# devarshpatel1506/Real-Time-Student-Attendance-System

Hardware: AMD Instinct MI355X
Metric: swipes/sec (fused BF.EXISTS+PFADD) at 1/2/4/8 GPUs; % of HBM peak (higher is better)
Workload: dtype u64; 1 GPU; c3-1B-10M-100kkeys; students=10000000, hll_keys_total=100000, hll_keys_this_gpu=100000, key_ownership=MurmurHash64A(key name, 0) mod world (distributed.KeyMap), id_bytes=8, parallelism=dp1 (key-sharded, Bloom replicated), k1_variant=partitioned, layout=offsets, streams=1, input=routed to the key owners at ingest, launch=host, answers=written (1 B per swipe)

## Files before the change

include/sketch.h:

```cpp
#ifndef SKETCH_H
#define SKETCH_H

#include <stddef.h>
#include <stdint.h>

#ifdef __cplusplus
extern "C" {
#endif

#define SKE_OK 0
#define SKE_EINVAL -1
#define SKE_ENOMEM -2
#define SKE_EHIP -3
#define SKE_ENOFILTER -4
#define SKE_EEXISTS -5
#define SKE_EFULL -6
#define SKE_ERANGE -7
#define SKE_EBADRATE -8
#define SKE_EBADCAP -9
#define SKE_EBADEXP -10
#define SKE_EBADHLL -11
#define SKE_ETOOLONG -12
#define SKE_EBUSY -13
#define SKE_ECMSNOKEY -14
// ... 261 lines not shown
    const uint32_t *slot;
    const uint8_t *bytes;
    const uint32_t *offs;
    uint32_t width;
    uint64_t n;
    uint8_t *out_valid;
} ske_swipe_batch;
int ske_swipes_many_async(ske_ctx *ctx, uint32_t fid, const ske_swipe_batch *batches,
                          uint32_t nbatch, uint32_t branches);
int ske_swipes_stats(ske_ctx *ctx, uint32_t fid, const uint8_t *bytes, const uint32_t *offs,
                     uint64_t n, uint64_t *probes, uint64_t *nvalid);
int ske_swipes_variant(ske_ctx *ctx, uint32_t fid);
int ske_set_option(ske_ctx *ctx, const char *name, int64_t value);
#define SKE_PASS_KINDS 9
int ske_pass_times(ske_ctx *ctx, double *ms_out, uint64_t *count_out, int reset);

typedef struct {
    uint8_t *status;
    uint32_t *id_start, *id_len, *lec_start, *lec_len, *ts_start, *ts_len;
    int32_t *day;
    uint64_t *kh;
} ske_ingest_cols_t;
int ske_ingest_parse(ske_ctx *ctx, const uint8_t *msgs, const uint32_t *moffs, uint64_t n,
                     int day_form, const ske_ingest_cols_t *cols);
int ske_keytab_lookup(ske_ctx *ctx, const ske_ingest_cols_t *cols, uint64_t n, uint32_t *slot_dev,
                      uint64_t *nmiss);
int ske_keytab_insert(ske_ctx *ctx, const uint64_t *kh_host, const uint32_t *slots_host, uint64_t n);
int ske_keytab_clear(ske_ctx *ctx);
int ske_ingest_swipes(ske_ctx *ctx, uint32_t fid, const uint8_t *msgs,
                      const ske_ingest_cols_t *cols, uint64_t n, uint8_t *valid_dev,
// ... 31 lines not shown
```

real-time-student-attendance-system_amd/_lib.py:

```python
from __future__ import annotations

import ctypes as C
import os

_HERE = os.path.dirname(os.path.abspath(__file__))
LIB_PATH = os.environ.get("SKE_LIB") or os.path.join(_HERE, "csrc", "libsketch.so")
HEADER_PATH = os.path.join(os.path.dirname(_HERE), "include", "sketch.h")

SKE_OK = 0
SKE_EINVAL = -1
SKE_ENOMEM = -2
SKE_EHIP = -3
SKE_ENOFILTER = -4
SKE_EEXISTS = -5
SKE_EFULL = -6
SKE_ERANGE = -7
SKE_EBADRATE = -8
SKE_EBADCAP = -9
SKE_EBADEXP = -10
SKE_EBADHLL = -11
SKE_ETOOLONG = -12
SKE_EBUSY = -13
SKE_ECMSNOKEY = -14
SKE_ECMSEXISTS = -15
# ... 199 lines not shown
    "ske_swipes_fixed_async": (C.c_int, [_CTX, C.c_uint32, _u32p, _u8p, C.c_uint32, C.c_uint64,
                                         _u8p]),
    "ske_swipes_many_async": (C.c_int, [_CTX, C.c_uint32, _vp, C.c_uint32, C.c_uint32]),
    "ske_swipes_fixed_bits": (C.c_int, [_CTX, C.c_uint32, _u32p, _u8p, C.c_uint32, C.c_uint64, _u8p, C.c_int]),
    "ske_route_swipes": (C.c_int, [_CTX, _u8p, C.c_uint32, _u32p, C.c_uint64, C.c_uint32, _u32p, _u32p,
                                   C.c_uint32, _u8p, _u32p, _u32p, _u64p]),
    "ske_route_swipes_cap_async": (C.c_int, [_CTX, _u8p, C.c_uint32, _u32p, C.c_uint64, C.c_uint32, _u32p,
                                             C.c_uint32, C.c_uint32, _u32p, _u8p, _u32p, _u32p, _u32p]),
    "ske_route_return_async": (C.c_int, [_CTX, _u8p, _u32p, C.c_uint64, _u8p]),
    "ske_route_slots_async": (C.c_int, [_CTX, _u32p, C.c_uint64, _u32p, C.c_uint32, C.c_uint32, _u32p]),
    "ske_swipes_stats": (C.c_int, [_CTX, C.c_uint32, _u8p, _u32p, C.c_uint64,
                                   C.POINTER(C.c_uint64), C.POINTER(C.c_uint64)]),
    "ske_swipes_variant": (C.c_int, [_CTX, C.c_uint32]),
    "ske_set_option": (C.c_int, [_CTX, C.c_char_p, C.c_int64]),
    "ske_pass_times": (C.c_int, [_CTX, C.POINTER(C.c_double), C.POINTER(C.c_uint64), C.c_int]),
    "ske_ingest_parse": (C.c_int, [_CTX, _u8p, _u32p, C.c_uint64, C.c_int, C.POINTER(IngestCols)]),
    "ske_keytab_lookup": (C.c_int, [_CTX, C.POINTER(IngestCols), C.c_uint64, _u32p,
                                    C.POINTER(C.c_uint64)]),
    "ske_keytab_insert": (C.c_int, [_CTX, _u64p, _u32p, C.c_uint64]),
    "ske_keytab_clear": (C.c_int, [_CTX]),
    "ske_ingest_swipes": (C.c_int, [_CTX, C.c_uint32, _u8p, C.POINTER(IngestCols), C.c_uint64, _u8p,
                                    C.POINTER(C.c_uint64)]),
    "ske_ingest_times": (C.c_int, [_CTX, _u8p, C.POINTER(IngestCols), C.c_uint64, _vp]),
    "ske_ingest_dense": (C.c_int, [_CTX, _u8p, C.POINTER(IngestCols), C.c_uint64, _u8p, _vp,
                                   C.POINTER(IngestDense), C.c_uint64, C.POINTER(C.c_uint64),
                                   C.POINTER(C.c_uint64)]),
    "ske_capture_begin": (C.c_int, [_CTX]),
    "ske_capture_end": (C.c_int, [_CTX, C.POINTER(C.c_void_p)]),
    "ske_graph_launch": (C.c_int, [_CTX, _vp]),
    "ske_graph_free": (C.c_int, [_CTX, _vp]),
# ... 75 lines not shown
```

real-time-student-attendance-system_amd/csrc/sketch_api_ctx.cpp:

```cpp
#include <stdlib.h>
#include <string.h>

#include "sketch_ctx.h"

using namespace ske;

namespace ske {

void *stage_buf(ske_ctx *c, StageSlot slot, size_t bytes, int *rc) {
    if (bytes < 64) bytes = 64;
    if (c->stg_cap[slot] < bytes) {
        if (c->stg[slot]) (void)hipFree(c->stg[slot]);
        c->stg[slot] = nullptr;
        c->stg_cap[slot] = 0;
        size_t want = bytes + bytes / 4 + 256;
        hipError_t e = hipMalloc(&c->stg[slot], want);
        if (e != hipSuccess) {
            c->last_hip = std::string("hipMalloc(staging): ") + hipGetErrorString(e);
            *rc = SKE_ENOMEM;
            return nullptr;
        }
        c->stg_cap[slot] = want;
    }
    return c->stg[slot];
// ... 388 lines not shown
        }
        mark_recycle(c, m);
    }
    c->marks.clear();
    for (int i = 0; i < kPassKinds; i++) {
        ms[i] = c->pass_ms[i];
        count[i] = c->pass_n[i];
        if (reset) {
            c->pass_ms[i] = 0;
            c->pass_n[i] = 0;
        }
    }
    return SKE_OK;
}

int ske_device_alloc(ske_ctx *c, uint64_t bytes, void **out) {
    if (!c || !out) return SKE_EINVAL;
    hipError_t e = hipMalloc(out, bytes ? bytes : 16);
    if (e != hipSuccess) {
        c->last_hip = std::string("hipMalloc: ") + hipGetErrorString(e);
        return SKE_ENOMEM;
    }
    return SKE_OK;
}

int ske_device_free(ske_ctx *c, void *p) {
    if (!c) return SKE_EINVAL;
    HIPCHK(c, hipFree(p));
    return SKE_OK;
}
// ... 12 lines not shown
int ske_set_option(ske_ctx *c, const char *name, int64_t value) {
    if (!c || !name) return SKE_EINVAL;
    static const struct {
        const char *name;
        int64_t min, max;
        void (*set)(ske_ctx *, int64_t);
    } options[] = {
        {"tile", 1, 8, [](ske_ctx *x, int64_t v) { x->pb = int(v); }},
        {"pass_timing", 0, 1, [](ske_ctx *x, int64_t v) { x->timing = v != 0; }},
        {"part_sub", 0, int64_t(1) << 26, [](ske_ctx *x, int64_t v) { x->part_sub = uint32_t(v); }},
        {"hll_seg", -1, 1, [](ske_ctx *x, int64_t v) { x->seg.mode = int(v); }},
        {"seg_density", 0, 1000000, [](ske_ctx *x, int64_t v) { x->seg.density_x100 = uint32_t(v); }},
        {"seg_dense_min", 0, 1000000, [](ske_ctx *x, int64_t v) { x->seg.dense_min_x100 = uint32_t(v); }},
        {"seg_klog", 0, 3, [](ske_ctx *x, int64_t v) { x->seg.klog = int(v); }},
        {"seg_b1", -1, 9, [](ske_ctx *x, int64_t v) { x->seg.b1 = int(v); }},
        {"k1_grid", 0, 65535, [](ske_ctx *x, int64_t v) { x->k1_grid = int(v); }},
        {"k1_persistent", 0, 1, [](ske_ctx *x, int64_t v) { x->k1_persistent = int(v); }},
        {"variant", -1, 3, [](ske_ctx *x, int64_t v) { x->variant = int(v); }},
    };
    for (const auto &o : options) {
        if (strcmp(name, o.name)) continue;
        if (value < o.min || value > o.max) return SKE_EINVAL;
        if (!strcmp(name, "tile") && (value & (value - 1))) return SKE_EINVAL;
        o.set(c, value);
        return SKE_OK;
    }
    return SKE_EINVAL;
}

int ske_capture_begin(ske_ctx *c) {
// ... 74 lines not shown
```

real-time-student-attendance-system_amd/csrc/sketch_internal.h:

```cpp
#pragma once
#include <cstddef>

#include "sketch_common.h"

namespace ske {

hipError_t launch_swipes(int mode, const ChainDev &ch, bool lds, int tile, const uint8_t *bytes,
                         const uint32_t *offs, uint32_t fixed_w, const uint32_t *slot, uint64_t n,
                         uint8_t *regs,
                         uint32_t nslots, uint8_t *out, unsigned long long *stats, int cus,
                         hipStream_t st);
hipError_t lds_bloom_setup();
hipError_t set_stamp_buffer(void *p);
uint32_t lds_bloom_max();
hipError_t launch_pfadd(const uint32_t *slot, const uint8_t *bytes, const uint32_t *offs,
                        uint64_t n, uint8_t *regs, uint32_t nslots, unsigned int *err, int cus,
                        hipStream_t st);
hipError_t launch_pfcount(const uint8_t *regs, const uint32_t *slots, const uint32_t *goffs,
                          uint32_t ngroups, const double *tau, const double *sig, uint64_t *out,
                          int cus, hipStream_t st);
hipError_t launch_histogram(const uint8_t *regs, uint32_t *out64, hipStream_t st);
hipError_t launch_pfmerge(uint8_t *regs, uint32_t dst, const uint32_t *srcs, uint32_t n,
                          hipStream_t st);
uint32_t pfmerge_partitions(uint32_t n, int cus, uint32_t *per);
// ... 113 lines not shown
                            uint32_t nslots, uint8_t *out, void *scratch, unsigned int *err,
                            int cus, int region_u, int finish_u, hipStream_t st);

constexpr int kPSliceLog = 19;
constexpr uint32_t kPSliceBits = 1u << kPSliceLog;
constexpr uint32_t kPMaxSlices = 2047;
constexpr int kPMaxLinks = 8;
struct Scratch;
bool part_supported(const ChainDev &ch);
struct SegOpts {
    int mode = -1;
    uint32_t density_x100 = 600;
    uint32_t dense_min_x100 = 100;
    int klog = 1;
    int b1 = -1;
};
hipError_t part_reserve(const ChainDev &ch, uint64_t n, uint32_t sub, uint32_t nslots, const SegOpts &so,
                        Scratch *scr);
typedef void (*PassHook)(void *user, int pass, int end, hipStream_t st);
struct PartBatch {
    const uint8_t *bytes;
    const uint32_t *offs;
    uint32_t fixed_w;
    const uint32_t *slot;
    uint64_t n;
    uint8_t *out;
};
hipError_t launch_swipes_part(const ChainDev &ch, const PartBatch *bt, uint32_t nb, uint8_t *regs,
                              uint32_t nslots, Scratch *scr, unsigned int *err, int cus, uint32_t sub,
                              const SegOpts &so, hipStream_t st, PassHook hook = nullptr,
// ... 120 lines not shown
hipError_t launch_tally_list(const TallyTab &T, uint64_t min_events, uint32_t cap, uint64_t *out_keys,
                             uint32_t *out_len, uint64_t *out_ev, uint64_t *out_va, unsigned int *out_n,
                             hipStream_t st);

hipError_t launch_hll_fmt_sizes(const uint8_t *regs, const uint32_t *slots, uint32_t nkeys, uint32_t nslots,
                                uint32_t smb, uint32_t *sizes, int cus, hipStream_t st);
hipError_t launch_hll_fmt_dump(const uint8_t *regs, const uint32_t *slots, uint32_t nkeys, uint32_t nslots,
                               uint32_t smb, const uint64_t *card, const uint32_t *offs, uint8_t *out, int cus,
                               hipStream_t st);
hipError_t launch_hll_fmt_load(uint8_t *regs, const uint32_t *slots, uint32_t nkeys, uint32_t nslots,
                               const uint8_t *blob, const uint32_t *offs, uint8_t *status, unsigned int *anybad,
                               int cus, hipStream_t st);
hipError_t launch_hll_fmt_offs_check(const uint32_t *offs, uint32_t n, unsigned int *bad, int cus, hipStream_t st);

struct Scratch;
constexpr int kScratchSlots = 48;

enum ScratchSlot : int {
    kScrKeysOrFirst,
    kScrKeysSorted,
    kScrVals,
    kScrValsSorted,
    kScrRank,
    kScrRankSorted,
    kScrPrefMax,
    kScrSortTmp,
    kScrScanKeyTmp,
    kScrScanTmp,
    kScrBfHa,
    kScrBfHb,
    kScrBfState,
// ... 18 lines not shown
    kScrPartRec,
    kScrPartOff,
    kScrPartFail,
    kScrPartHllw,
    kScrPartFlist,
    kScrSegR1,
    kScrSegFill,
    kScrSegCtab,
    kScrSegR2,
    kScrSegO2,
    kScrSegCb,
    kScrSegQ,
    kScrSegQitems,
    kScrSegMlist,
    kScrSegCopies,
    kScrRouteHist,
    kScrRouteTot,
    kScratchSlotCount
};
static_assert(kScratchSlotCount <= kScratchSlots, "Scratch holds kScratchSlots slots");

enum StageSlot : int {
    kStgBytes,
    kStgOffs,
    kStgSlots,
    kStgOut,
    kStgAnswers,
    kStgReply,
    kStgList,
    kStgList2,
// ... 10 lines not shown
    kStgHllFmtBlob,
    kStgHllFmtStatus,
    kStgHllFmtFlag,
    kStgTallyFlag,
    kStgTallyMask,
    kStgTallyKeys,
    kStgTallyLen,
    kStgTallyEv,
    kStgTallyVa,
    kStageSlotCount
};

Scratch *scratch_new();
void scratch_delete(Scratch *s);
void *scratch_get(Scratch *s, ScratchSlot slot, size_t bytes, hipError_t *err);
void scratch_set_recording(Scratch *s, bool on);
void scratch_unpin(Scratch *s);

hipError_t pfadd_exact(Scratch *s, const uint32_t *slot, const uint8_t *bytes,
                       const uint32_t *offs, uint64_t n, uint8_t *regs, uint32_t nslots,
                       uint8_t *changed_dev, unsigned int *err_dev, int cus, hipStream_t st);

hipError_t launch_bf_hash(const uint8_t *bytes, const uint32_t *offs, uint64_t n, uint64_t *ha,
                          uint64_t *hb, int cus, hipStream_t st);
hipError_t launch_bf_settle_present(const ChainDev &ch, uint64_t n, const uint64_t *ha,
                                    const uint64_t *hb, uint8_t *state, int8_t *res, int cus,
                                    hipStream_t st);
hipError_t launch_bf_first_setter(const LinkDev &L, uint64_t n, const uint64_t *ha,
                                  const uint64_t *hb, const uint8_t *state, uint32_t *first,
                                  int cus, hipStream_t st);
// ... 22 lines not shown
```

real-time-student-attendance-system_amd/csrc/sketch_order.hip:

```cpp
#include <rocprim/device/device_radix_sort.hpp>
#include <rocprim/device/device_scan.hpp>
#include <rocprim/device/device_scan_by_key.hpp>

#include "sketch_common.h"
#include "sketch_internal.h"

namespace ske {

struct Scratch {
    void *p[kScratchSlots] = {};
    size_t cap[kScratchSlots] = {};
    bool recording = false;
    bool pinned[kScratchSlots] = {};
};

void scratch_set_recording(Scratch *s, bool on) { s->recording = on; }
void scratch_unpin(Scratch *s) {
    for (int i = 0; i < kScratchSlots; i++) s->pinned[i] = false;
}

void *scratch_get(Scratch *s, ScratchSlot slot, size_t bytes, hipError_t *err) {
    if (bytes == 0) bytes = 16;
    if (s->recording) s->pinned[slot] = true;
    if (s->cap[slot] < bytes && s->pinned[slot]) {
// ... 2 lines not shown
    }
    if (s->cap[slot] < bytes) {
        if (s->p[slot]) (void)hipFree(s->p[slot]);
        s->p[slot] = nullptr;
        s->cap[slot] = 0;
        size_t want = bytes + bytes / 4 + 256;
        hipError_t e = hipMalloc(&s->p[slot], want);
        if (e != hipSuccess) {
            *err = e;
            return nullptr;
        }
        s->cap[slot] = want;
    }
    return s->p[slot];
}

void scratch_free_all(Scratch *s) {
    for (int i = 0; i < kScratchSlots; i++)
        if (s->p[i]) (void)hipFree(s->p[i]);
}

Scratch *scratch_new() { return new Scratch(); }
void scratch_delete(Scratch *s) {
    scratch_free_all(s);
    delete s;
}

static inline unsigned grid_for(uint64_t n, unsigned block, unsigned cap) {
    uint64_t g = (n + block - 1) / block;
    if (g < 1) g = 1;
// ... 296 lines not shown
```

real-time-student-attendance-system_amd/csrc/sketch_part.h:

```cpp
#pragma once
#include "sketch_common.h"
#include "sketch_internal.h"
#include "sketch_seg_plan.h"

namespace ske {

constexpr uint32_t kPSub = 1u << 26;
constexpr uint32_t kPbGroup = 8;
constexpr uint32_t kPbLanes = 64 / kPbGroup;
constexpr uint32_t kPTileLog = 10;
constexpr uint32_t kPTile = 1u << kPTileLog;

struct PartLink {
    const uint8_t *bf;
    uint64_t m;
    uint32_t d;
    uint32_t t;
    uint32_t sh;
    uint32_t k;
    uint32_t slice0;
    uint32_t nbytes16;
};

struct PartArgs {
// ... 102 lines not shown
    uint32_t s;
    uint32_t nsub;
    uint32_t maxch;
    uint32_t nwin;
    uint32_t dense_min;
    uint32_t *q;
    uint4 *qitems;
    uint4 *mlist;
    uint8_t *copies;
    uint32_t ccap;
    uint32_t *fill;
    uint32_t *ctab;
    uint32_t kmaxc;
    uint32_t kstat;
    unsigned int *err;
};

inline bool part_flist(const PartArgs &A) { return A.nlinks == 1 && A.ksum == 11 && A.nslices <= 2046; }

bool seg_use(const PartArgs &A, const SegOpts &so, uint32_t nslots, uint64_t n, uint32_t sub, SegPlan *P);
hipError_t seg_scratch(const SegPlan &P, uint32_t sub, uint64_t n, Scratch *scr, SegArgs *S);
hipError_t launch_seg_sub(const PartArgs &A, SegArgs &S, const SegPlan &P, uint32_t si, int cus, hipStream_t st,
                          PassHook hook, void *hook_user);
hipError_t launch_seg_windows(PartArgs A, SegArgs S, const SegPlan &P, uint32_t ns, int cus, hipStream_t st,
                              PassHook hook, void *hook_user);

}
```

real-time-student-attendance-system_amd/csrc/sketch_seg.hip:

```cpp
#include <algorithm>
#include <type_traits>

#include "sketch_part.h"
#include "sketch_seg_plan.h"

namespace ske {

__device__ __forceinline__ uint32_t seg_scan(uint32_t v, uint32_t *ws, uint32_t &total) {
    const uint32_t tid = threadIdx.x, lane = tid & 63, wave = tid >> 6, nw = blockDim.x >> 6;
    const uint32_t inc = part_wave_scan(v);
    lds_barrier();
    if (lane == 63) ws[wave] = inc;
    lds_barrier();
    uint32_t pre = 0, tot = 0;
    for (uint32_t w = 0; w < nw; w++) {
        const uint32_t x = ws[w];
        pre += w < wave ? x : 0;
        tot += x;
    }
    total = tot;
    return pre + inc - v;
}

__device__ __forceinline__ uint32_t seg_last_le(const uint32_t *a, uint32_t n, uint32_t v) {
// ... 183 lines not shown
                    for (uint32_t e = 0; e < 4; e++) {
                        if (j + e >= total) break;
                        const uint32_t h = m[e] & (kSegMaxB1 - 1), i = j + e + cnt[h];
                        S.r1[size_t(slot_of(i, slt[h])) * kSegChunk + (i & (kSegChunk - 1))] = v[e];
                    }
                }
            }
            if (tid < S.nb1)
                for (uint32_t k = cv; k < cvp; k++)
                    S.r1[size_t(slot_of(abase + k, aslot)) * kSegChunk + ((abase + k) & (kSegChunk - 1))] = 0u;
        }
        lds_barrier();
    }
}

constexpr uint32_t kSegDT = 512;
template <uint32_t T> struct SegDA {
    static constexpr uint32_t R = kSegChunk / T;
    static constexpr uint32_t BPC = 3;
    static constexpr uint32_t WPE = BPC * (T / 64) / 4;
    static_assert(T == 512, "three blocks per CU");
};
template <uint32_t T>
__global__ void __launch_bounds__(T, SegDA<T>::WPE) k_seg_da(const SegArgs S) {
    constexpr uint32_t R = SegDA<T>::R;
    static_assert(R % 4 == 0 && kSegMaxWpb <= T && kSegMaxB1 <= T, "D geometry");
    __shared__ uint32_t tot[kSegMaxB1], cbl[kSegMaxB1 + 1];
    __shared__ uint32_t c2[kSegMaxWpb + 1];
    __shared__ __attribute__((aligned(16))) uint32_t sb[kSegChunk];
    __shared__ uint32_t ws[T / 64];
    const uint32_t tid = threadIdx.x, wpb = 1u << S.wlog;
    const uint32_t *fl = S.fill + seg_fill_at(S, 0);
    uint32_t t = 0;
    if (tid < S.nb1) {
        t = fl[tid * kSegFillStride];
        tot[tid] = t;
    }
    uint32_t nqa;
    const uint32_t cbase = seg_scan(tid < S.nb1 ? (t + kSegChunk - 1) / kSegChunk : 0u, ws, nqa);
    const uint32_t nq = nqa < S.maxch ? nqa : S.maxch;
    if (tid < S.nb1) {
        cbl[tid] = cbase;
        if (blockIdx.x == 0) S.cb[size_t(S.s) * (S.nb1 + 1) + tid] = cbase < S.maxch ? cbase : S.maxch;
    }
    if (tid == 0 && blockIdx.x == 0) {
        S.cb[size_t(S.s) * (S.nb1 + 1) + S.nb1] = nq;
// ... 16 lines not shown
        const uint32_t w0 = c * kSegChunk, th = tot[h];
        const uint32_t n = th - w0 < kSegChunk ? th - w0 : kSegChunk;
        uint32_t rec[R];
#pragma unroll
        for (uint32_t k = 0; k < R / 4; k++) {
            const uint32_t x = (k * T + tid) * 4;
            const part_u32x4 v = __builtin_bit_cast(
                part_u32x4, __builtin_amdgcn_raw_buffer_load_b128(rr1, x < n ? (p * kSegChunk + x) * 4 : kOOR, 0,
                                                                  kNt2Aux<2>));
            rec[4 * k] = v.x;
            rec[4 * k + 1] = v.y;
            rec[4 * k + 2] = v.z;
            rec[4 * k + 3] = v.w;
        }
        for (uint32_t j = tid; j <= wpb; j += T) c2[j] = 0;
        lds_barrier();
        uint32_t pos[R];
#pragma unroll
        for (uint32_t j = 0; j < R; j++) {
            pos[j] = 0xffffffffu;
            if ((j / 4 * T + tid) * 4 + j % 4 < n && (rec[j] & 63u) != 0) {
                const uint32_t w2 = (rec[j] >> (kSegRecShift + S.klog)) & (wpb - 1);
                pos[j] = (w2 << 16) | atomicAdd(&c2[w2], 1u);
            }
        }
        lds_barrier();
        uint32_t total;
        const uint32_t ex = seg_scan(tid < wpb ? c2[tid] : 0u, ws, total);
        if (tid < wpb) {
            c2[tid] = ex;
            o2[size_t(q) * (wpb + 1) + tid] = ex;
        }
        if (tid == 0) o2[size_t(q) * (wpb + 1) + wpb] = total;
        lds_barrier();
#pragma unroll
        for (uint32_t j = 0; j < R; j++)
            if (pos[j] != 0xffffffffu) sb[c2[pos[j] >> 16] + (pos[j] & 0xffffu)] = rec[j];
        lds_barrier();
        part_u32x4 *dst = reinterpret_cast<part_u32x4 *>(r2 + size_t(q) * kSegChunk);
        const part_u32x4 *src = reinterpret_cast<const part_u32x4 *>(sb);
        for (uint32_t j = tid; j * 4 < total; j += T) nt2_st<4>(dst + j, src[j]);
    }
}

__device__ __forceinline__ bool seg_lds_max(uint32_t *w, uint32_t sh, uint32_t rank) {
    uint32_t old = *w;
    while (((old >> sh) & 0xffu) < rank) {
        const uint32_t prev = atomicCAS(w, old, (old & ~(0xffu << sh)) | (rank << sh));
        if (prev == old) return true;
        old = prev;
    }
    return false;
}

#ifdef SKE_SEG_STAMPS
__device__ unsigned long long *ske_seg_stamp_buf;
// ... 33 lines not shown
template <int KLOG, bool QUEUE>
__global__ void __launch_bounds__(SegE<KLOG>::T, SegE<KLOG>::WPS) k_seg_e(const PartArgs A, const SegArgs S) {
    using E = SegE<KLOG>;
    constexpr uint32_t T = E::T;
    constexpr uint32_t KW = 1u << KLOG, WB = KW << kHllP, NPC = WB / 16 / T;
    constexpr uint32_t NL = KW * (kHllRegs / 128);
    constexpr uint32_t RPT = E::RPT, EP = E::EP;
    constexpr uint32_t SLICE = seg_slice(KLOG);
    __shared__ __attribute__((aligned(16))) uint8_t win[WB];
    __shared__ uint8_t dirty[NL];
    __shared__ uint32_t rb[EP], rp[EP + 1];
    __shared__ uint32_t spre[2][65], cq0[2][64], ws[T / 64], hdr[2];
    const uint32_t tid = threadIdx.x, lane = tid & 63, wave = tid >> 6;
    const uint32_t nb1m = S.nb1 - 1;
    const uint32_t nitems = QUEUE ? S.q[0] : S.nwin;
    const __amdgpu_buffer_rsrc_t rr2 = part_rsrc(S.r2, S.nsub * S.maxch * kSegChunk * 4);
    uint32_t cq = 0, cc = 0;
    uint32_t pbase = 0, plen = 0, pnp = 0;
    auto item = [&](uint32_t it, uint32_t &wi, uint32_t &sl, uint32_t &copy) {
        wi = it;
        sl = 0;
        copy = 0xffffffffu;
        if (QUEUE) {
            const uint4 e = S.qitems[it];
            wi = e.x;
            sl = e.y;
            copy = e.z;
        }
    };
    auto p1 = [&](uint32_t wi) {
        const uint32_t h = wi & nb1m;
        if (tid < S.nsub) {
            cq = S.cb[size_t(tid) * (S.nb1 + 1) + h];
            cc = S.cb[size_t(tid) * (S.nb1 + 1) + h + 1];
        }
    };
    auto image = [&](uint32_t wi) {
        const uint32_t slot0 = wi << KLOG;
        const uint32_t nk = A.nslots - slot0 < KW ? A.nslots - slot0 : KW;
        const __amdgpu_buffer_rsrc_t r = part_rsrc(A.regs + (size_t(slot0) << kHllP), nk << kHllP);
#pragma unroll
        for (uint32_t i = 0; i < NPC; i++) {
            const uint32_t piece = i * (T / 64) + wave;
            __builtin_amdgcn_raw_ptr_buffer_load_lds(
                r, (__attribute__((address_space(3))) void *)(win + piece * 1024), 16,
                int(piece * 1024 + lane * 16), 0, 0, kNt2Aux<16>);
        }
    };
    const uint32_t orow = (1u << S.wlog) + 1;
// ... 17 lines not shown
        if (tid < EP && tid < pnp) plen = run_of(pb, tid, wi >> S.b1, pbase);
    };
    uint32_t it = blockIdx.x, par = 0;
    uint32_t wi_n = 0, sl_n = 0, copy_n = 0;
    if (it < nitems) {
        item(it, wi_n, sl_n, copy_n);
        p1(wi_n);
        p2(0, wi_n);
        image(wi_n);
    }
    uint32_t nit = 0;
    for (; it < nitems; it = nit, par ^= 1) {
        const uint32_t wi = wi_n, sl = sl_n;
        uint32_t copy = copy_n;
        const uint32_t np = pnp;
        const uint32_t stamp = QUEUE ? S.nwin + it : wi;
        (void)stamp;
        SEG_STAMP(stamp, 0, 0);
        const uint32_t w2 = wi >> S.b1;
        const uint32_t slot0 = wi << KLOG;
        const uint32_t nk = A.nslots - slot0 < KW ? A.nslots - slot0 : KW;
        uint8_t *g = A.regs + (size_t(slot0) << kHllP);
        const uint32_t npc = nk << (kHllP - 4);
        uint32_t nrec, nrec0;
        {
            const uint32_t ex = seg_scan(plen, ws, nrec0);
            if (tid < EP) {
                rb[tid] = pbase;
                rp[tid] = ex;
            }
// ... 12 lines not shown
            if (tid == 0) {
                uint32_t base = atomicAdd(&S.q[1], nsl);
                if (base + nsl > S.ccap) {
                    base = 0xffffffffu;
                } else {
                    const uint32_t qp = atomicAdd(&S.q[0], nsl - 1);
                    for (uint32_t k = 1; k < nsl; k++) S.qitems[qp + k - 1] = make_uint4(wi, k, base + k, 0);
                    S.mlist[atomicAdd(&S.q[2], 1u)] = make_uint4(wi, base, nsl, 0);
                }
                hdr[0] = base;
            }
            lds_barrier();
            copy = hdr[0];
        }
        const bool cut = copy != 0xffffffffu;
        const uint32_t lo = cut ? sl * SLICE : 0;
        const uint32_t hi = cut ? (nrec - lo < SLICE ? nrec : lo + SLICE) : nrec;
        const bool dense = nrec > 0 && (cut || nrec >= S.dense_min);
        if (dense)
            for (uint32_t j = tid; j < NL; j += T) dirty[j] = 0;
        if (tid == 0)
            hdr[1] = QUEUE || gridDim.x < kPGroups
                         ? gridDim.x + atomicAdd(&S.q[QUEUE ? 5 : 4], 1u)
                         : gridDim.x + kPGroups * atomicAdd(&S.q[8 + blockIdx.x % kPGroups], 1u) +
                               blockIdx.x % kPGroups;
        __syncthreads();
        nit = hdr[1];
        if (nit < nitems) {
            item(nit, wi_n, sl_n, copy_n);
            p1(wi_n);
// ... 80 lines not shown
        if (nit < nitems) image(wi_n);
        SEG_STAMP(stamp, 4, uint64_t(nrec) | (uint64_t(np) << 32) | (uint64_t(dense) << 63));
    }
}

__device__ __forceinline__ part_u32x4 seg_max16(part_u32x4 a, part_u32x4 b) {
    typedef unsigned char u8x16 __attribute__((ext_vector_type(16)));
    return __builtin_bit_cast(part_u32x4,
                              __builtin_elementwise_max(__builtin_bit_cast(u8x16, a), __builtin_bit_cast(u8x16, b)));
}

template <int KLOG>
__global__ void __launch_bounds__(1024) k_seg_m(const PartArgs A, const SegArgs S) {
    constexpr uint32_t KW = 1u << KLOG, WB = KW << kHllP;
    const uint32_t nm = S.q[2];
    for (uint32_t m = blockIdx.x; m < nm; m += gridDim.x) {
        const uint4 e = S.mlist[m];
        const uint32_t slot0 = e.x << KLOG;
        const uint32_t nk = A.nslots - slot0 < KW ? A.nslots - slot0 : KW;
        part_u32x4 *g = reinterpret_cast<part_u32x4 *>(A.regs + (size_t(slot0) << kHllP));
        for (uint32_t j = threadIdx.x; j < (nk << (kHllP - 4)); j += 1024) {
            part_u32x4 v = reinterpret_cast<const part_u32x4 *>(S.copies + size_t(e.y) * WB)[j];
            for (uint32_t c = 1; c < e.z; c++)
                v = seg_max16(v, reinterpret_cast<const part_u32x4 *>(S.copies + size_t(e.y + c) * WB)[j]);
            g[j] = v;
        }
    }
}


// ... 13 lines not shown
    S->r1 = (uint32_t *)scratch_get(scr, kScrSegR1, size_t(L.r1_slots) * kSegChunk * 4, &e);
    if (e == hipSuccess)
        S->fill = (uint32_t *)scratch_get(scr, kScrSegFill, size_t(P.nsub) * (P.nb1 + 1) * kSegFillStride * 4, &e);
    if (e == hipSuccess) S->ctab = (uint32_t *)scratch_get(scr, kScrSegCtab, size_t(P.nb1) * S->kmaxc * 4, &e);
    if (e == hipSuccess)
        S->r2 = (uint32_t *)scratch_get(scr, kScrSegR2, size_t(L.rows) * kSegChunk * 4, &e);
    if (e == hipSuccess)
        S->o2 = (uint32_t *)scratch_get(scr, kScrSegO2, size_t(L.rows) * ((1u << P.wlog) + 1) * 4, &e);
    if (e == hipSuccess) S->cb = (uint32_t *)scratch_get(scr, kScrSegCb, size_t(P.nsub) * (P.nb1 + 1) * 4, &e);
    const uint32_t ccap = uint32_t(2 * ((mg + seg_slice(P.klog) - 1) / seg_slice(P.klog)) + 2);
    const size_t wb = size_t(1) << (P.klog + kHllP);
    if (e == hipSuccess) S->q = (uint32_t *)scratch_get(scr, kScrSegQ, 64, &e);
    if (e == hipSuccess) S->qitems = (uint4 *)scratch_get(scr, kScrSegQitems, size_t(ccap) * 16, &e);
    if (e == hipSuccess) S->mlist = (uint4 *)scratch_get(scr, kScrSegMlist, size_t(ccap) * 16, &e);
    if (e == hipSuccess) S->copies = (uint8_t *)scratch_get(scr, kScrSegCopies, size_t(ccap) * wb, &e);
    S->ccap = ccap;
    S->nb1 = P.nb1;
    S->s1 = P.s1;
    S->b1 = P.b1;
    S->wlog = P.wlog;
    S->klog = P.klog;
    S->nsub = P.nsub;
    S->maxch = P.maxch;
    S->nwin = P.nwin;
    S->dense_min = P.dense_min;
    return e;
}

hipError_t launch_seg_sub(const PartArgs &A, SegArgs &S, const SegPlan &P, uint32_t si, int cus, hipStream_t st,
                          PassHook hook, void *hook_user) {
    if (hook) hook(hook_user, 2, 0, st);
    S.s = si % P.nsub;
    S.err = A.err;
    S.nruns = (A.ntiles + kSegRunTiles - 1) / kSegRunTiles;
    if (S.s == 0) {
        hipError_t e = hipMemsetAsync(S.fill, 0, size_t(P.nsub) * (P.nb1 + 1) * kSegFillStride * 4, st);
        if (e == hipSuccess) e = hipMemsetAsync(S.ctab, 0, size_t(P.nb1) * S.kmaxc * 4, st);
        if (e != hipSuccess) return e;
    }
    hipLaunchKernelGGL(k_seg_c1<kSegC1T>, dim3(std::min(S.nruns, unsigned(cus) * SegC1<kSegC1T>::BPC)), dim3(kSegC1T),
                       0, st, A, S);
    if (hook) hook(hook_user, 2, 1, st);
    if (hook) hook(hook_user, 3, 0, st);
    hipLaunchKernelGGL(k_seg_da<kSegDT>, dim3(unsigned(cus) * SegDA<kSegDT>::BPC), dim3(kSegDT), 0, st, S);
    if (hook) hook(hook_user, 3, 1, st);
    return hipGetLastError();
}

template <int K> static void seg_e_launch(const PartArgs &A, const SegArgs &S, int cus, hipStream_t st) {
    hipLaunchKernelGGL((k_seg_e<K, false>), dim3(unsigned(cus) * SegE<K>::BPC), dim3(SegE<K>::T), 0, st, A, S);
    hipLaunchKernelGGL((k_seg_e<K, true>), dim3(unsigned(cus) * SegE<K>::BPC), dim3(SegE<K>::T), 0, st, A, S);
    hipLaunchKernelGGL(k_seg_m<K>, dim3(unsigned(cus)), dim3(1024), 0, st, A, S);
}
// ... 19 lines not shown
```

real-time-student-attendance-system_amd/csrc/sketch_seg_plan.h:

```cpp
#pragma once
#include <algorithm>
#include <cstdint>

#include "sketch_internal.h"

namespace ske {

constexpr uint32_t kSegChunk = 8192;
constexpr uint32_t kSegRun = 8192;

struct SegPlan {
    uint32_t s1, b1, wlog, klog, nb1, nwin, maxch, nsub, dense_min;
};

inline uint64_t seg_fill_max(uint32_t nb1, uint64_t sub) {
    const uint64_t full = sub / kSegRun, tail = sub % kSegRun;
    return full * (kSegRun + 3 * std::min<uint64_t>(nb1, kSegRun)) + tail + 3 * std::min<uint64_t>(nb1, tail);
}

inline uint32_t seg_rows_max(uint32_t nb1, uint64_t sub) {
    return uint32_t((seg_fill_max(nb1, sub) + uint64_t(nb1) * (kSegChunk - 4)) / kSegChunk);
}

inline bool seg_plan(uint32_t nslots, uint64_t n, uint32_t sub, const SegOpts &so, SegPlan *P) {
    if (nslots == 0 || n == 0 || so.klog < 0 || so.klog > 3) return false;
    const uint32_t klog = uint32_t(so.klog);
    const uint32_t nwin = uint32_t((uint64_t(nslots) + (1u << klog) - 1) >> klog);
// ... 14 lines not shown
    }
    if (wlog > 9) return false;
    P->klog = klog;
    P->wlog = wlog;
    P->b1 = b1;
    P->s1 = klog + wlog;
    P->nwin = nwin;
    P->nb1 = 1u << b1;
    P->maxch = seg_rows_max(P->nb1, sub);
    const uint64_t kmax = ((uint64_t(1) << 29) - 1) / (uint64_t(P->maxch) * kSegChunk);
    const uint64_t ns = (n + sub - 1) / sub;
    if (kmax == 0) return false;
    P->nsub = uint32_t(std::min<uint64_t>(std::min<uint64_t>(ns, kmax), 64));
    const uint64_t dm = uint64_t(so.dense_min_x100) * ((uint64_t(1) << klog) * (kHllRegs / 128)) / 100;
    P->dense_min = dm < 1 ? 1u : (dm > 0xffffffffu ? 0xffffffffu : uint32_t(dm));
    return true;
}

struct SegSlots {
    uint32_t kstat, kmaxc, dyn;
    uint32_t r1_slots;
    uint64_t rows;
};
inline SegSlots seg_slots(const SegPlan &P, uint32_t sub, uint64_t n) {
    const uint64_t m = n < sub ? n : sub;
    const uint64_t ch = (m + kSegChunk - 1) / kSegChunk, dyn = ch + P.nb1;
    uint64_t kst = 2 * ((ch + P.nb1 - 1) / P.nb1) + 2;
    kst = std::min<uint64_t>(kst, ((1u << 14) - 1 - dyn) / P.nb1);
    SegSlots L;
    L.kstat = uint32_t(kst);
// ... 9 lines not shown
```

real-time-student-attendance-system_amd/engine.py:

```python
from __future__ import annotations

import ctypes as C
import gc

import numpy as np

from ._lib import (CmsInfo, Context, GenParams, HhInfo, HhStats, IngestDense, SKE_HH_ID_BYTES, SKE_HLL_DUMP_CARD,
                   SKE_MEM_DEVICE, SKE_MEM_HOST, SKE_TALLY_KEY_BYTES, SKE_TP_BINS, TallyInfo)
from . import synthetic

PASS_KINDS = 9


class _no_gc:

    def __enter__(self):
        gc.collect()
        self.was = gc.isenabled()
        gc.disable()

    def __exit__(self, *exc):
        if self.was:
            gc.enable()
        return False
# ... 289 lines not shown
                      b.n, C.byref(probes), C.byref(nvalid))
        return probes.value, nvalid.value

    def variant(self, fid: int) -> int:
        return self.ctx.lib.ske_swipes_variant(self.ctx.ptr, fid)

    def set_option(self, name: str, value: int):
        self.ctx.call("ske_set_option", name.encode(), int(value))

    def pass_times(self, reset: bool = True) -> list[tuple[float, int]]:
        ms = (C.c_double * PASS_KINDS)()
        cnt = (C.c_uint64 * PASS_KINDS)()
        self.ctx.call("ske_pass_times", ms, cnt, 1 if reset else 0)
        return [(ms[i], cnt[i]) for i in range(PASS_KINDS)]

    def set_stream(self, stream_ptr: int | None):
        self.ctx.call("ske_set_stream", C.c_void_p(stream_ptr) if stream_ptr else None)

    def get_stream(self) -> int | None:
        p = C.c_void_p()
        self.ctx.call("ske_get_stream", C.byref(p))
        return p.value

    def sync(self):
        self.ctx.call("ske_sync")

    def check_errors(self):
        self.ctx.call("ske_check_errors")

    def cms_init(self, cid: int, width: int, depth: int):
# ... 213 lines not shown
```

Baseline: 32.67 billion swipes/s.

## Drop HLL updates that cannot raise register floor on hot windows

After: 33.91 billion swipes/s (median of 6 runs). +3.8%, better.

```diff
diff --git a/include/sketch.h b/include/sketch.h
--- a/include/sketch.h
+++ b/include/sketch.h
@@ -299,6 +299,7 @@
 int ske_set_option(ske_ctx *ctx, const char *name, int64_t value);
 #define SKE_PASS_KINDS 9
 int ske_pass_times(ske_ctx *ctx, double *ms_out, uint64_t *count_out, int reset);
+int ske_seg_floor_stats(ske_ctx *ctx, uint64_t out[3]);
 
 typedef struct {
     uint8_t *status;
diff --git a/real-time-student-attendance-system_amd/_lib.py b/real-time-student-attendance-system_amd/_lib.py
--- a/real-time-student-attendance-system_amd/_lib.py
+++ b/real-time-student-attendance-system_amd/_lib.py
@@ -237,6 +237,7 @@
     "ske_swipes_variant": (C.c_int, [_CTX, C.c_uint32]),
     "ske_set_option": (C.c_int, [_CTX, C.c_char_p, C.c_int64]),
     "ske_pass_times": (C.c_int, [_CTX, C.POINTER(C.c_double), C.POINTER(C.c_uint64), C.c_int]),
+    "ske_seg_floor_stats": (C.c_int, [_CTX, C.POINTER(C.c_uint64)]),
     "ske_ingest_parse": (C.c_int, [_CTX, _u8p, _u32p, C.c_uint64, C.c_int, C.POINTER(IngestCols)]),
     "ske_keytab_lookup": (C.c_int, [_CTX, C.POINTER(IngestCols), C.c_uint64, _u32p,
                                     C.POINTER(C.c_uint64)]),
diff --git a/real-time-student-attendance-system_amd/csrc/sketch_api_ctx.cpp b/real-time-student-attendance-system_amd/csrc/sketch_api_ctx.cpp
--- a/real-time-student-attendance-system_amd/csrc/sketch_api_ctx.cpp
+++ b/real-time-student-attendance-system_amd/csrc/sketch_api_ctx.cpp
@@ -426,6 +426,18 @@
     return SKE_OK;
 }
 
+int ske_seg_floor_stats(ske_ctx *c, uint64_t out[3]) {
+    if (!c || !out) return SKE_EINVAL;
+    out[0] = out[1] = out[2] = 0;
+    void *p = scratch_peek(c->scratch, kScrSegFstat);
+    if (!p) return SKE_OK;
+    if (c->xr.stream && c->xr.stream != c->st) HIPCHK(c, hipStreamSynchronize(c->xr.stream));
+    HIPCHK(c, hipMemcpyAsync(out, p, 3 * sizeof(uint64_t), hipMemcpyDeviceToHost, c->st));
+    HIPCHK(c, hipMemsetAsync(p, 0, 3 * sizeof(uint64_t), c->st));
+    HIPCHK(c, hipStreamSynchronize(c->st));
+    return SKE_OK;
+}
+
 int ske_device_alloc(ske_ctx *c, uint64_t bytes, void **out) {
     if (!c || !out) return SKE_EINVAL;
     hipError_t e = hipMalloc(out, bytes ? bytes : 16);
@@ -468,6 +480,8 @@
         {"seg_dense_min", 0, 1000000, [](ske_ctx *x, int64_t v) { x->seg.dense_min_x100 = uint32_t(v); }},
         {"seg_klog", 0, 3, [](ske_ctx *x, int64_t v) { x->seg.klog = int(v); }},
         {"seg_b1", -1, 9, [](ske_ctx *x, int64_t v) { x->seg.b1 = int(v); }},
+        {"seg_floor", 0, 1, [](ske_ctx *x, int64_t v) { x->seg.floor = int(v); }},
+        {"seg_hot_min", 0, int64_t(1) << 31, [](ske_ctx *x, int64_t v) { x->seg.hot_min = uint32_t(v); }},
         {"k1_grid", 0, 65535, [](ske_ctx *x, int64_t v) { x->k1_grid = int(v); }},
         {"k1_persistent", 0, 1, [](ske_ctx *x, int64_t v) { x->k1_persistent = int(v); }},
         {"variant", -1, 3, [](ske_ctx *x, int64_t v) { x->variant = int(v); }},
diff --git a/real-time-student-attendance-system_amd/csrc/sketch_internal.h b/real-time-student-attendance-system_amd/csrc/sketch_internal.h
--- a/real-time-student-attendance-system_amd/csrc/sketch_internal.h
+++ b/real-time-student-attendance-system_amd/csrc/sketch_internal.h
@@ -151,6 +151,8 @@
     uint32_t dense_min_x100 = 100;
     int klog = 1;
     int b1 = -1;
+    int floor = 1;
+    uint32_t hot_min = 4096;
 };
 hipError_t part_reserve(const ChainDev &ch, uint64_t n, uint32_t sub, uint32_t nslots, const SegOpts &so,
                         Scratch *scr);
@@ -301,7 +303,7 @@
 hipError_t launch_hll_fmt_offs_check(const uint32_t *offs, uint32_t n, unsigned int *bad, int cus, hipStream_t st);
 
 struct Scratch;
-constexpr int kScratchSlots = 48;
+constexpr int kScratchSlots = 52;
 
 enum ScratchSlot : int {
     kScrKeysOrFirst,
@@ -350,6 +352,9 @@
     kScrSegQitems,
     kScrSegMlist,
     kScrSegCopies,
+    kScrSegFloor,
+    kScrSegHot,
+    kScrSegFstat,
     kScrRouteHist,
     kScrRouteTot,
     kScratchSlotCount
@@ -390,6 +395,8 @@
 Scratch *scratch_new();
 void scratch_delete(Scratch *s);
 void *scratch_get(Scratch *s, ScratchSlot slot, size_t bytes, hipError_t *err);
+void *scratch_get_zeroed(Scratch *s, ScratchSlot slot, size_t bytes, hipError_t *err);
+void *scratch_peek(const Scratch *s, ScratchSlot slot);
 void scratch_set_recording(Scratch *s, bool on);
 void scratch_unpin(Scratch *s);
 
diff --git a/real-time-student-attendance-system_amd/csrc/sketch_order.hip b/real-time-student-attendance-system_amd/csrc/sketch_order.hip
--- a/real-time-student-attendance-system_amd/csrc/sketch_order.hip
+++ b/real-time-student-attendance-system_amd/csrc/sketch_order.hip
@@ -40,6 +40,22 @@
     }
     return s->p[slot];
 }
+
+void *scratch_get_zeroed(Scratch *s, ScratchSlot slot, size_t bytes, hipError_t *err) {
+    const void *was = s->p[slot];
+    const size_t cap = s->cap[slot];
+    void *p = scratch_get(s, slot, bytes, err);
+    if (p && (p != was || s->cap[slot] != cap)) {
+        const hipError_t e = hipMemset(p, 0, s->cap[slot]);
+        if (e != hipSuccess) {
+            *err = e;
+            return nullptr;
+        }
+    }
+    return p;
+}
+
+void *scratch_peek(const Scratch *s, ScratchSlot slot) { return s->p[slot]; }
 
 void scratch_free_all(Scratch *s) {
     for (int i = 0; i < kScratchSlots; i++)
diff --git a/real-time-student-attendance-system_amd/csrc/sketch_part.h b/real-time-student-attendance-system_amd/csrc/sketch_part.h
--- a/real-time-student-attendance-system_amd/csrc/sketch_part.h
+++ b/real-time-student-attendance-system_amd/csrc/sketch_part.h
@@ -140,7 +140,14 @@
     uint32_t kmaxc;
     uint32_t kstat;
     unsigned int *err;
+    uint8_t *floor;
+    uint8_t *hot;
+    unsigned long long *fstat;
+    uint32_t hot_min;
 };
+constexpr uint32_t kSegHotHdr = 16;
+constexpr uint32_t kSegHotMagic = 0x686f7431u;
+constexpr uint32_t kSegHotAge = 4;
 
 inline bool part_flist(const PartArgs &A) { return A.nlinks == 1 && A.ksum == 11 && A.nslices <= 2046; }
 
diff --git a/real-time-student-attendance-system_amd/csrc/sketch_seg.hip b/real-time-student-attendance-system_amd/csrc/sketch_seg.hip
--- a/real-time-student-attendance-system_amd/csrc/sketch_seg.hip
+++ b/real-time-student-attendance-system_amd/csrc/sketch_seg.hip
@@ -221,6 +221,73 @@
     }
 }
 
+__device__ __forceinline__ bool seg_hot_valid(const SegArgs &S) {
+    const uint32_t *h = reinterpret_cast<const uint32_t *>(S.hot);
+    return h[0] == S.nwin && h[1] == S.klog && h[2] == S.b1 && h[3] == kSegHotMagic;
+}
+__device__ __forceinline__ uint32_t seg_floor_at(const SegArgs &S, uint32_t w, uint32_t k) {
+    return ((w & (S.nb1 - 1)) << S.s1) | ((w >> S.b1) << S.klog) | k;
+}
+__device__ __forceinline__ part_u32x4 seg_min16(part_u32x4 a, part_u32x4 b) {
+    typedef unsigned char u8x16 __attribute__((ext_vector_type(16)));
+    return __builtin_bit_cast(part_u32x4,
+                              __builtin_elementwise_min(__builtin_bit_cast(u8x16, a), __builtin_bit_cast(u8x16, b)));
+}
+__device__ __forceinline__ uint32_t seg_wave_min8(part_u32x4 v) {
+    uint32_t x = 0xffu;
+#pragma unroll
+    for (uint32_t c = 0; c < 4; c++)
+#pragma unroll
+        for (uint32_t sh = 0; sh < 32; sh += 8) {
+            const uint32_t y = (v[c] >> sh) & 0xffu;
+            x = x < y ? x : y;
+        }
+#pragma unroll
+    for (int o = 32; o > 0; o >>= 1) {
+        const uint32_t z = uint32_t(__shfl_xor(int(x), o));
+        x = x < z ? x : z;
+    }
+    return x;
+}
+constexpr uint32_t kSegFloorHead = 4;
+constexpr uint32_t kSegFT = 256;
+__global__ void __launch_bounds__(kSegFT) k_seg_floor(const uint8_t *regs, uint32_t nslots, const SegArgs S) {
+    __shared__ uint32_t nfl;
+    const uint32_t tid = threadIdx.x, lane = tid & 63;
+    const uint32_t nwaves = gridDim.x * (kSegFT / 64), gw = blockIdx.x * (kSegFT / 64) + (tid >> 6);
+    if (tid == 0) nfl = 0;
+    __syncthreads();
+    uint8_t *hot = S.hot + kSegHotHdr;
+    uint32_t mine = 0;
+    if (seg_hot_valid(S)) {
+        for (uint32_t w0 = gw; w0 < S.nwin; w0 += nwaves * 64) {
+            const uint32_t wl = w0 + lane * nwaves;
+            const uint32_t hv = wl < S.nwin ? hot[wl] : 0u;
+            if (hv) hot[wl] = uint8_t((hv < kSegHotAge ? hv : kSegHotAge) - 1);
+            for (uint64_t m = __ballot(hv != 0); m; m &= m - 1) {
+                const uint32_t w = w0 + uint32_t(__builtin_ctzll(m)) * nwaves;
+                mine++;
+                for (uint32_t k = 0; k < (1u << S.klog); k++) {
+                    const uint32_t slot = (w << S.klog) | k;
+                    if (slot >= nslots) break;
+                    const part_u32x4 *p = reinterpret_cast<const part_u32x4 *>(regs + (size_t(slot) << kHllP));
+                    part_u32x4 v = p[lane];
+#pragma unroll
+                    for (uint32_t i = 1; i < kSegFloorHead; i++) v = seg_min16(v, p[i * 64 + lane]);
+                    if (seg_wave_min8(v) == 0) continue;
+#pragma unroll
+                    for (uint32_t i = kSegFloorHead; i < (kHllRegs / 16) / 64; i++) v = seg_min16(v, p[i * 64 + lane]);
+                    const uint32_t x = seg_wave_min8(v);
+                    if (lane == 0) S.floor[seg_floor_at(S, w, k)] = uint8_t(x);
+                }
+            }
+        }
+    }
+    if (lane == 0 && mine) atomicAdd(&nfl, mine);
+    __syncthreads();
+    if (tid == 0 && nfl) atomicAdd(S.fstat, (unsigned long long)nfl);
+}
+
 constexpr uint32_t kSegDT = 512;
 template <uint32_t T> struct SegDA {
     static constexpr uint32_t R = kSegChunk / T;
@@ -236,7 +303,12 @@
     __shared__ uint32_t c2[kSegMaxWpb + 1];
     __shared__ __attribute__((aligned(16))) uint32_t sb[kSegChunk];
     __shared__ uint32_t ws[T / 64];
+    __shared__ __attribute__((aligned(16))) uint8_t fls[kSegMaxWpb * 8];
+    __shared__ uint32_t nst[2];
     const uint32_t tid = threadIdx.x, wpb = 1u << S.wlog;
+    const bool ff = S.floor != nullptr;
+    uint32_t nsaw = 0, ndrop = 0;
+    if (tid < 2) nst[tid] = 0;
     const uint32_t *fl = S.fill + seg_fill_at(S, 0);
     uint32_t t = 0;
     if (tid < S.nb1) {
@@ -283,14 +355,29 @@
             rec[4 * k + 3] = v.w;
         }
         for (uint32_t j = tid; j <= wpb; j += T) c2[j] = 0;
+        if (ff) {
+            const uint8_t *fb = S.floor + (size_t(h) << S.s1);
+            if (S.s1 >= 4) {
+                if (tid < (1u << (S.s1 - 4)))
+                    reinterpret_cast<part_u32x4 *>(fls)[tid] = reinterpret_cast<const part_u32x4 *>(fb)[tid];
+            } else if (tid < (1u << S.s1)) {
+                fls[tid] = fb[tid];
+            }
+        }
         lds_barrier();
         uint32_t pos[R];
 #pragma unroll
         for (uint32_t j = 0; j < R; j++) {
             pos[j] = 0xffffffffu;
             if ((j / 4 * T + tid) * 4 + j % 4 < n && (rec[j] & 63u) != 0) {
-                const uint32_t w2 = (rec[j] >> (kSegRecShift + S.klog)) & (wpb - 1);
-                pos[j] = (w2 << 16) | atomicAdd(&c2[w2], 1u);
+                const uint32_t f = ff ? fls[rec[j] >> kSegRecShift] : 0u;
+                nsaw++;
+                if ((rec[j] & 63u) > f) {
+                    const uint32_t w2 = (rec[j] >> (kSegRecShift + S.klog)) & (wpb - 1);
+                    pos[j] = (w2 << 16) | atomicAdd(&c2[w2], 1u);
+                } else {
+                    ndrop++;
+                }
             }
         }
         lds_barrier();
@@ -309,6 +396,12 @@
         part_u32x4 *dst = reinterpret_cast<part_u32x4 *>(r2 + size_t(q) * kSegChunk);
         const part_u32x4 *src = reinterpret_cast<const part_u32x4 *>(sb);
         for (uint32_t j = tid; j * 4 < total; j += T) nt2_st<4>(dst + j, src[j]);
+    }
+    if (ff) {
+        if (nsaw) atomicAdd(&nst[0], nsaw);
+        if (ndrop) atomicAdd(&nst[1], ndrop);
+        __syncthreads();
+        if (tid < 2 && nst[tid]) atomicAdd(S.fstat + 1 + tid, (unsigned long long)nst[tid]);
     }
 }
 
@@ -372,9 +465,11 @@
     const uint32_t tid = threadIdx.x, lane = tid & 63, wave = tid >> 6;
     const uint32_t nb1m = S.nb1 - 1;
     const uint32_t nitems = QUEUE ? S.q[0] : S.nwin;
+    const bool hinting = !QUEUE && S.hot != nullptr, hot_ok = hinting && seg_hot_valid(S);
     const __amdgpu_buffer_rsrc_t rr2 = part_rsrc(S.r2, S.nsub * S.maxch * kSegChunk * 4);
     uint32_t cq = 0, cc = 0;
     uint32_t pbase = 0, plen = 0, pnp = 0;
+    uint32_t hint_n = 0, floor_n = 0;
     auto item = [&](uint32_t it, uint32_t &wi, uint32_t &sl, uint32_t &copy) {
         wi = it;
         sl = 0;
@@ -391,6 +486,14 @@
         if (tid < S.nsub) {
             cq = S.cb[size_t(tid) * (S.nb1 + 1) + h];
             cc = S.cb[size_t(tid) * (S.nb1 + 1) + h + 1];
+        }
+        if (hinting && tid == 0) {
+            hint_n = hot_ok ? S.hot[kSegHotHdr + wi] : 0u;
+            floor_n = 0;
+            for (uint32_t k = 0; k < KW && (wi << KLOG) + k < A.nslots; k++) {
+                const uint32_t fk = S.floor[seg_floor_at(S, wi, k)];
+                floor_n = fk > floor_n ? fk : floor_n;
+            }
         }
     };
     auto image = [&](uint32_t wi) {
@@ -438,6 +541,7 @@
         const uint32_t wi = wi_n, sl = sl_n;
         uint32_t copy = copy_n;
         const uint32_t np = pnp;
+        const uint32_t hv = hint_n, fw = floor_n;
         const uint32_t stamp = QUEUE ? S.nwin + it : wi;
         (void)stamp;
         SEG_STAMP(stamp, 0, 0);
@@ -480,6 +584,14 @@
             copy = hdr[0];
         }
         const bool cut = copy != 0xffffffffu;
+        if (hinting && tid == 0) {
+            uint32_t nv = hv;
+            if (nrec) {
+                const uint64_t est = uint64_t(nrec) << (fw < 31 ? fw : 31), thr = uint64_t(S.hot_min) * nk;
+                nv = cut || est >= thr ? kSegHotAge : (2 * est < thr ? 0u : (hv ? kSegHotAge : 0u));
+            }
+            if (nv != hv || !hot_ok) S.hot[kSegHotHdr + wi] = uint8_t(nv);
+        }
         const uint32_t lo = cut ? sl * SLICE : 0;
         const uint32_t hi = cut ? (nrec - lo < SLICE ? nrec : lo + SLICE) : nrec;
         const bool dense = nrec > 0 && (cut || nrec >= S.dense_min);
@@ -590,6 +702,13 @@
 __global__ void __launch_bounds__(1024) k_seg_m(const PartArgs A, const SegArgs S) {
     constexpr uint32_t KW = 1u << KLOG, WB = KW << kHllP;
     const uint32_t nm = S.q[2];
+    if (S.hot != nullptr && blockIdx.x == 0 && threadIdx.x == 0) {
+        uint32_t *h = reinterpret_cast<uint32_t *>(S.hot);
+        h[0] = S.nwin;
+        h[1] = S.klog;
+        h[2] = S.b1;
+        h[3] = kSegHotMagic;
+    }
     for (uint32_t m = blockIdx.x; m < nm; m += gridDim.x) {
         const uint4 e = S.mlist[m];
         const uint32_t slot0 = e.x << KLOG;
@@ -633,6 +752,15 @@
     if (e == hipSuccess) S->qitems = (uint4 *)scratch_get(scr, kScrSegQitems, size_t(ccap) * 16, &e);
     if (e == hipSuccess) S->mlist = (uint4 *)scratch_get(scr, kScrSegMlist, size_t(ccap) * 16, &e);
     if (e == hipSuccess) S->copies = (uint8_t *)scratch_get(scr, kScrSegCopies, size_t(ccap) * wb, &e);
+    S->floor = nullptr;
+    S->hot = nullptr;
+    S->fstat = nullptr;
+    S->hot_min = P.hot_min;
+    if (P.floor) {
+        if (e == hipSuccess) S->floor = (uint8_t *)scratch_get(scr, kScrSegFloor, size_t(P.nb1) << P.s1, &e);
+        if (e == hipSuccess) S->hot = (uint8_t *)scratch_get_zeroed(scr, kScrSegHot, kSegHotHdr + size_t(P.nwin), &e);
+        if (e == hipSuccess) S->fstat = (unsigned long long *)scratch_get_zeroed(scr, kScrSegFstat, 3 * 8, &e);
+    }
     S->ccap = ccap;
     S->nb1 = P.nb1;
     S->s1 = P.s1;
@@ -655,7 +783,10 @@
     if (S.s == 0) {
         hipError_t e = hipMemsetAsync(S.fill, 0, size_t(P.nsub) * (P.nb1 + 1) * kSegFillStride * 4, st);
         if (e == hipSuccess) e = hipMemsetAsync(S.ctab, 0, size_t(P.nb1) * S.kmaxc * 4, st);
+        if (e == hipSuccess && S.floor) e = hipMemsetAsync(S.floor, 0, size_t(P.nb1) << P.s1, st);
         if (e != hipSuccess) return e;
+        if (S.floor)
+            hipLaunchKernelGGL(k_seg_floor, dim3(unsigned(cus) * 4), dim3(kSegFT), 0, st, A.regs, A.nslots, S);
     }
     hipLaunchKernelGGL(k_seg_c1<kSegC1T>, dim3(std::min(S.nruns, unsigned(cus) * SegC1<kSegC1T>::BPC)), dim3(kSegC1T),
                        0, st, A, S);
diff --git a/real-time-student-attendance-system_amd/csrc/sketch_seg_plan.h b/real-time-student-attendance-system_amd/csrc/sketch_seg_plan.h
--- a/real-time-student-attendance-system_amd/csrc/sketch_seg_plan.h
+++ b/real-time-student-attendance-system_amd/csrc/sketch_seg_plan.h
@@ -11,6 +11,7 @@
 
 struct SegPlan {
     uint32_t s1, b1, wlog, klog, nb1, nwin, maxch, nsub, dense_min;
+    uint32_t floor, hot_min;
 };
 
 inline uint64_t seg_fill_max(uint32_t nb1, uint64_t sub) {
@@ -55,6 +56,8 @@
     P->nsub = uint32_t(std::min<uint64_t>(std::min<uint64_t>(ns, kmax), 64));
     const uint64_t dm = uint64_t(so.dense_min_x100) * ((uint64_t(1) << klog) * (kHllRegs / 128)) / 100;
     P->dense_min = dm < 1 ? 1u : (dm > 0xffffffffu ? 0xffffffffu : uint32_t(dm));
+    P->floor = so.floor != 0;
+    P->hot_min = so.hot_min;
     return true;
 }
 
diff --git a/real-time-student-attendance-system_amd/engine.py b/real-time-student-attendance-system_amd/engine.py
--- a/real-time-student-attendance-system_amd/engine.py
+++ b/real-time-student-attendance-system_amd/engine.py
@@ -327,6 +327,11 @@
         self.ctx.call("ske_pass_times", ms, cnt, 1 if reset else 0)
         return [(ms[i], cnt[i]) for i in range(PASS_KINDS)]
 
+    def seg_floor_stats(self) -> tuple[int, int, int]:
+        out = (C.c_uint64 * 3)()
+        self.ctx.call("ske_seg_floor_stats", out)
+        return int(out[0]), int(out[1]), int(out[2])
+
     def set_stream(self, stream_ptr: int | None):
         self.ctx.call("ske_set_stream", C.c_void_p(stream_ptr) if stream_ptr else None)
 
```
